# vita-epfl/collaborative-gan-sampling

Hardware: AMD Instinct MI355X
Metric: refined samples/sec @ 20 refinement steps (higher is better)
Workload: dtype f32; 1 GPU; dcgan64 collaborative refinement (propose + K-step refine + render), batch 1024/GPU, K=20, momentum rate 0.1, refine at feature [8, 8, 256], random-init weights, z~U(-1,1) seed 2019+rank; global_batch=1024, refine_steps=20, parallelism=single GPU, hipgraph=True, batches_in_flight=2, fused_per_launch=1, sync_bn=False, contraction=f32

## Files before the change

collaborative-gan-sampling_amd/csrc/api.hip:

```cpp
#include <stdarg.h>
#include <stdio.h>

#include "cgs_internal.h"

static thread_local char g_err[512] = "";
static thread_local const char* g_last_kernel = "";

static thread_local double g_last_flops = 0.0;
static thread_local int g_last_tail[2] = {0, 0};
void cgs_note_tail(int tiles, int split) { g_last_tail[0] = tiles; g_last_tail[1] = split; }
static thread_local int g_contraction = CGS_CONTRACTION_F32;
int cgs_contraction_mode() { return g_contraction; }

void cgs_note_kernel(const char* name) { g_last_kernel = name; }
void cgs_note_flops(double f) { g_last_flops = f; }
void cgs_add_flops(double f) { g_last_flops += f; }

int cgs_set_error(int code, const char* fmt, ...) {
    va_list ap;
    va_start(ap, fmt);
    vsnprintf(g_err, sizeof(g_err), fmt, ap);
    va_end(ap);
    return code;
}

extern "C" {

int cgs_version(void) { return 111; }
const char* cgs_last_error(void) { return g_err; }
const char* cgs_last_kernel(void) { return g_last_kernel; }
double cgs_last_executed_flops(void) { return g_last_flops; }
int cgs_last_tail_tiles(void) { return g_last_tail[0]; }
int cgs_last_tail_split(void) { return g_last_tail[1]; }
int cgs_set_contraction(int mode) {
    if (mode < CGS_CONTRACTION_F32 || mode > CGS_CONTRACTION_BX6_ALL) return cgs_set_error(CGS_EINVAL, "set_contraction: mode %d", mode);
    g_contraction = mode;
    return CGS_OK;
}
int cgs_get_contraction(void) { return g_contraction; }

}

struct ConvCall { CgsLayer L; bool dirT, deconv, bwd; };

static ConvCall conv_call_of(int op, int H, int W, int Cin, int Ho, int Wo, int Cout, int kh, int kw, int sh, int sw) {
    ConvCall c;
    c.deconv = (op == CGS_DECONV_FWD || op == CGS_DECONV_BWD_DATA);
    c.bwd = (op == CGS_CONV_BWD_DATA || op == CGS_DECONV_BWD_DATA);
    c.dirT = (op == CGS_CONV_BWD_DATA || op == CGS_DECONV_FWD);
    CgsLayer& L = c.L;
    L.kh = kh; L.kw = kw; L.sh = sh; L.sw = sw;
    if (!c.deconv) { L.Hb = H; L.Wb = W; L.Cb = Cin; L.Hs = cgs_ceil_div(H, sh > 0 ? sh : 1); L.Ws = cgs_ceil_div(W, sw > 0 ? sw : 1); L.Cs = Cout; }
    else { L.Hs = H; L.Ws = W; L.Cs = Cin; L.Hb = Ho; L.Wb = Wo; L.Cb = Cout; }
    return c;
}

static int check_layer(const CgsLayer& L, const char* who) {
    if (L.kh <= 0 || L.kw <= 0 || L.sh <= 0 || L.sw <= 0 || L.Hb <= 0 || L.Wb <= 0 || L.Cb <= 0 || L.Cs <= 0)
        return cgs_set_error(CGS_EINVAL, "%s: non-positive dimension", who);
    if (L.Hs != cgs_ceil_div(L.Hb, L.sh) || L.Ws != cgs_ceil_div(L.Wb, L.sw))
        return cgs_set_error(CGS_EINVAL, "%s: 'SAME' geometry mismatch: big %dx%d stride %dx%d needs small %dx%d, got %dx%d", who,
                             L.Hb, L.Wb, L.sh, L.sw, cgs_ceil_div(L.Hb, L.sh), cgs_ceil_div(L.Wb, L.sw), L.Hs, L.Ws);
    return CGS_OK;
}

static IgemmParams igemm_geometry(const CgsLayer& L, bool dirT, int B, int epilogue) {
    IgemmParams p{};
    p.B = B; p.epilogue = epilogue;
    if (!dirT) cgs_geom_F(L, p);
    else if (L.sh <= 2 && L.sw <= 2) cgs_geom_T(L, p);
    return p;
}

static size_t in_image_floats(const IgemmParams& p) { return (size_t)p.Hin * p.Win * p.Cred; }
static size_t out_image_floats(const IgemmParams& p) { return (size_t)p.Hout * p.Wout * p.N; }
static size_t images_per_launch(const IgemmParams& p) {
    const size_t in_img = in_image_floats(p) * 4, out_img = out_image_floats(p) * 4;
    return 0x7fffffffUL / (in_img > out_img ? in_img : out_img);
}
static bool whole_batch_in_one_launch(const IgemmParams& p) { return images_per_launch(p) >= (size_t)p.B; }

// ... 429 lines not shown
```

collaborative-gan-sampling_amd/csrc/igemm.hip:

```cpp
#include <stdarg.h>
#include <stdio.h>

#include "cgs_internal.h"
#include "igemm_epilogue.h"

typedef float f32x16 __attribute__((ext_vector_type(16)));

static constexpr int BK = CGS_BK;

void cgs_geom_F(const CgsLayer& L, IgemmParams& p) {
    p.Hin = L.Hb; p.Win = L.Wb; p.Cred = L.Cb;
    p.Hout = L.Hs; p.Wout = L.Ws; p.N = L.Cs; p.Np = cgs_round_up(L.Cs, 64);
    p.S = L.sh; p.So = 1; p.dstep = 1; p.kstep = 1; p.nclasses = 1;
    p.tap_parity = (L.sh == 2 && L.sw == 2 && L.Hs * L.Ws > 64) ? 1 : 0;
    IgemmClass& c = p.cls[0];
    c.R = L.Hs; c.C = L.Ws; c.py = 0; c.px = 0; c.nty = L.kh; c.ntx = L.kw;
    c.dy0 = -cgs_same_pad_before(L.Hb, L.kh, L.sh); c.dx0 = -cgs_same_pad_before(L.Wb, L.kw, L.sw);
    c.ky0 = 0; c.kx0 = 0; c.K = L.kh * L.kw * L.Cb; c.w_off = 0;
    p.vec = (p.Cred % BK) == 0 && c.nty <= 16 && c.ntx <= 16;
}

void cgs_geom_T(const CgsLayer& L, IgemmParams& p) {
    p.Hin = L.Hs; p.Win = L.Ws; p.Cred = L.Cs;
    p.Hout = L.Hb; p.Wout = L.Wb; p.N = L.Cb; p.Np = cgs_round_up(L.Cb, 64);
// ... 22 lines not shown

size_t cgs_packed_floats(const IgemmParams& p) {
    size_t n = 0;
    for (int i = 0; i < p.nclasses; ++i) n += (size_t)cgs_round_up(p.cls[i].K, BK) * p.Np;
    return n;
}

__global__ void pack_weights_kernel(IgemmParams p, const float* __restrict__ w, float* __restrict__ packed,
                                    int kw, int Cb, int Cs, int dirT) {
    const IgemmClass& c = p.cls[blockIdx.y];
    const int Kpad = (c.K + BK - 1) / BK * BK;
    const size_t total = (size_t)Kpad * p.Np;
    for (size_t i = (size_t)blockIdx.x * blockDim.x + threadIdx.x; i < total; i += (size_t)gridDim.x * blockDim.x) {
        const int e = (int)(i & 3);
        const int n = (int)((i >> 2) % p.Np);
        const int k = (int)((i >> 2) / p.Np) * 4 + e;
        float v = 0.f;
        if (k < c.K && n < p.N) {
            int t, ci, ta, tb;
            if (p.vec) {
                const int ntaps = c.nty * c.ntx;
                const int kt = k / BK, chunk = kt / ntaps;
                t = kt - chunk * ntaps; ci = chunk * BK + (k - kt * BK);
                ta = t / c.ntx; tb = t - ta * c.ntx;
                ta = cgs_tap_order(ta, c.nty, p.tap_parity); tb = cgs_tap_order(tb, c.ntx, p.tap_parity);
            } else {
                t = k / p.Cred; ci = k - t * p.Cred;
                ta = t / c.ntx; tb = t - ta * c.ntx;
            }
            const int tap = (c.ky0 + ta * p.kstep) * kw + (c.kx0 + tb * p.kstep);
            const size_t src = dirT ? ((size_t)tap * Cb + n) * Cs + ci
                                    : ((size_t)tap * Cb + ci) * Cs + n;
            v = w[src];
        }
        packed[c.w_off + i] = v;
    }
}

int cgs_pack_weights(const IgemmParams& p, const CgsLayer& L, bool dirT, const float* w, float* packed, hipStream_t s) {
    size_t mx = 0;
    for (int i = 0; i < p.nclasses; ++i) {
        size_t n = (size_t)cgs_round_up(p.cls[i].K, BK) * p.Np;
        if (n > mx) mx = n;
    }
    if (mx == 0) return CGS_OK;
    int blocks = (int)((mx + 255) / 256);
    if (blocks > 4096) blocks = 4096;
    hipLaunchKernelGGL(pack_weights_kernel, dim3(blocks, p.nclasses), dim3(256), 0, s, p, w, packed, L.kw, L.Cb, L.Cs,
                       dirT ? 1 : 0);
    CGS_CHECK_LAUNCH("pack_weights");
    return CGS_OK;
}

template <int BM, int BN, int NW, bool VEC, int TBK, bool PAR, bool NS>
__device__ __forceinline__ void igemm_body(const IgemmParams& p) {
    constexpr int BK = TBK;
    constexpr int LDA = BK + 4;
    constexpr int NT = 64 * NW;
    constexpr int WM = BM / 64;
    constexpr int WN = NW / WM;
    constexpr int TM = BM / (32 * WM), TN = BN / (32 * WN);
    constexpr int QPR = BK / 4;
    constexpr int AI = BM * QPR / NT, BI = BN * QPR / NT;
    constexpr int AR = NT / QPR;
    extern __shared__ __attribute__((aligned(16))) float smem[];
    float* As = smem;
    float* Bs = smem + 2 * BM * LDA;
    constexpr int KLOOP_F = 2 * BM * LDA + 2 * BK * BN;
    constexpr int EH = (VEC && TBK == 16) ? 2 : 1;
    constexpr int STAGE_F = NW * (BM / WM / EH) * (BN / WN + 4);
    int* rowpix = (int*)(smem + (KLOOP_F > STAGE_F ? KLOOP_F : STAGE_F));

    const int nblk_n = p.Np / BN;
    unsigned wi = blockIdx.x;
    int cls_i = blockIdx.y;
    if (p.xcd_map == 2) {
        const unsigned xcd = wi & 7u;
        unsigned q = wi >> 3;
        cls_i = (int)(q % (unsigned)p.nclasses);
        q /= (unsigned)p.nclasses;
        wi = (q << 3) | xcd;
    }
    if (p.cls_flip && (((((unsigned)blockIdx.z * gridDim.y + (unsigned)cls_i) * gridDim.x) >> 8) & 1u)) {
        const int grp = cls_i / p.cls_flip;
        cls_i = grp * p.cls_flip + (p.cls_flip - 1 - (cls_i - grp * p.cls_flip));
    }
    int tsplit = 1, tz = 0, ttile = 0;
    if (p.tail_s > 1 && cls_i == p.nclasses - 1 && wi >= (unsigned)p.tail_from) {
        const unsigned t = wi - (unsigned)p.tail_from;
        ttile = (int)(t / (unsigned)p.tail_s); tz = (int)(t - (unsigned)ttile * (unsigned)p.tail_s); tsplit = p.tail_s;
        if (ttile >= p.tail_n) return;
        wi = (unsigned)p.tail_from + (unsigned)ttile;
    }
    int nb, mb;
    if (p.xcd_map) {
        const unsigned xcd = wi & 7u, q = wi >> 3;
        nb = (int)(q % (unsigned)nblk_n);
        mb = (int)(q / (unsigned)nblk_n) * 8 + (int)xcd;
    } else {
        nb = (int)(wi % (unsigned)nblk_n);
        mb = (int)(wi / (unsigned)nblk_n);
    }
    const IgemmClass& c = p.cls[cls_i];
    const int RC = c.R * c.C;
    const int M = p.B * RC;
    if (mb * BM >= M) return;
    if (p.lpt) {
        const int gpp = p.B / BM;
// ... 77 lines not shown
        return kt < nk ? kt : nk;
    };

    f32x4 ra[AI], rb[BI];
    const __amdgpu_buffer_rsrc_t in_rsrc = __builtin_amdgcn_make_buffer_rsrc(
        (void*)p.in, 0, (int)((unsigned)p.B * (unsigned)p.Hin * (unsigned)p.Win * (unsigned)p.Cred * 4u), 0x00020000);
#define LOAD_TILE(kt_)                                                                                          \
    do {                                                                                                        \
        if constexpr (VEC) {                                                                                    \
            const int kt32_ = TBK == 16 ? (kt_) >> 1 : (kt_);             \
            const int chunk_ = kt32_ / ntaps, t = kt32_ - chunk_ * ntaps;                                       \
            const int ci = chunk_ * 32 + (TBK == 16 ? ((kt_) & 1) * 16 : 0) + aq * 4;                           \
            const int ia_ = t / c.ntx, ib_ = t - ia_ * c.ntx;                                                   \
            const int ta = cgs_tap_order(ia_, c.nty, PAR), tb = cgs_tap_order(ib_, c.ntx, PAR);                 \
            const int dy = ta * p.dstep, dx = tb * p.dstep;                                                     \
            _Pragma("unroll") for (int i = 0; i < AI; ++i) {                                                    \
                const int iy = a_iy[i] + dy, ix = a_ix[i] + dx;                                                 \
                const bool ok = (unsigned)iy < (unsigned)p.Hin && (unsigned)ix < (unsigned)p.Win;               \
                  \
                                              \
                const unsigned off = ok ? (unsigned)((a_base[i] + iy * p.Win + ix) * p.Cred + ci) * 4u : 0xFFFFFFF0u; \
                ra[i] = __builtin_bit_cast(f32x4, __builtin_amdgcn_raw_buffer_load_b128(in_rsrc, off, 0, 0));   \
            }                                                                                                   \
        } else {                                                                                                \
               \
                                    \
            float va[AI][4];                                                                                    \
            _Pragma("unroll") for (int e = 0; e < 4; ++e) {                                                     \
                const int k = (kt_) * BK + aq * 4 + e;                                                          \
                const bool kin = k < c.K;                                                                       \
                const int t = kin ? k / p.Cred : 0, ci = k - t * p.Cred;                                        \
                const int ta = t / c.ntx, tb = t - ta * c.ntx;                                                  \
                const int dy = ta * p.dstep, dx = tb * p.dstep;                                                 \
                _Pragma("unroll") for (int i = 0; i < AI; ++i) {                                                \
                    const int iy = a_iy[i] + dy, ix = a_ix[i] + dx;                                             \
                    const bool ok = kin && (unsigned)iy < (unsigned)p.Hin && (unsigned)ix < (unsigned)p.Win;    \
                    const unsigned off = ok ? (unsigned)((a_base[i] + iy * p.Win + ix) * p.Cred + ci) * 4u : 0xFFFFFFF0u; \
                    va[i][e] = __builtin_bit_cast(float, __builtin_amdgcn_raw_buffer_load_b32(in_rsrc, off, 0, 0)); \
                }                                                                                               \
            }                                                                                                   \
            _Pragma("unroll") for (int i = 0; i < AI; ++i) ra[i] = f32x4{va[i][0], va[i][1], va[i][2], va[i][3]}; \
        }                                                                                                       \
        _Pragma("unroll") for (int i = 0; i < BI; ++i) {                                                        \
            const int idx = tid + NT * i;                                                                       \
            const int kq = idx / BN, n = idx - kq * BN;                                                         \
            rb[i] = *(const f32x4*)(wsrc + ((size_t)((kt_) * (BK / 4) + kq) * p.Np + n0 + n) * 4);            \
        }                                                                                                       \
    } while (0)
#define STORE_TILE(buf_)                                                                                        \
    do {                                                                                                        \
        float* a_ = As + (buf_) * BM * LDA;                                                                     \
        float* b_ = Bs + (buf_) * BK * BN;                                                                      \
        _Pragma("unroll") for (int i = 0; i < AI; ++i) *(f32x4*)(a_ + (ar + AR * i) * LDA + aq * 4) = ra[i];    \
        _Pragma("unroll") for (int i = 0; i < BI; ++i) *(f32x4*)(b_ + (tid + NT * i) * 4) = rb[i];              \
    } while (0)

    f32x16 acc[TM][TN];
#pragma unroll
    for (int tm = 0; tm < TM; ++tm)
#pragma unroll
        for (int tn = 0; tn < TN; ++tn)
#pragma unroll
            for (int r = 0; r < 16; ++r) acc[tm][tn][r] = 0.f;

    struct KIt { int kt, sub, ia, ib, chunk; };
    auto kit_valid = [&](const KIt& s) -> bool {
        if (!skip_ok) return true;
        const int ta = cgs_tap_order(s.ia, c.nty, PAR), tb = cgs_tap_order(s.ib, c.ntx, PAR);
        const int iy = u_iy + ta * p.dstep, ix = u_ix + tb * p.dstep;
        return (unsigned)iy < (unsigned)p.Hin && (unsigned)ix < (unsigned)p.Win;
    };
    auto kit_next_tap = [&](KIt& s) {
        for (;;) {
            if (++s.ib == c.ntx) { s.ib = 0; if (++s.ia == c.nty) { s.ia = 0; ++s.chunk; } }
            if (s.kt >= nk || kit_valid(s)) break;
            s.kt += (TBK == 16 ? 2 : 1);
        }
        if (s.kt > nk) s.kt = nk;
    };
    auto kit_first = [&](int kt0) -> KIt {
        KIt s;
        const int kt32 = (VEC && TBK == 16) ? kt0 >> 1 : kt0;
        s.kt = kt0; s.sub = (VEC && TBK == 16) ? (kt0 & 1) : 0;
        s.chunk = kt32 / ntaps;
        const int t = kt32 - s.chunk * ntaps;
        s.ia = t / c.ntx; s.ib = t - s.ia * c.ntx;
        if (s.kt < nk && !kit_valid(s)) {
            s.kt += (TBK == 16 ? 2 - s.sub : 1); s.sub = 0;
            kit_next_tap(s);
        }
        if (s.kt > nk) s.kt = nk;
        return s;
    };
    auto kit_next = [&](KIt s) -> KIt {
        if (TBK == 16 && s.sub == 0) { s.sub = 1; ++s.kt; if (s.kt > nk) s.kt = nk; return s; }
        s.sub = 0; ++s.kt;
        kit_next_tap(s);
        return s;
    };
    unsigned rowoff[AI], b_voff[BI];
#pragma unroll
    for (int i = 0; i < AI; ++i)
        rowoff[i] = ((unsigned)(a_base[i] + a_iy[i] * p.Win + a_ix[i]) * (unsigned)p.Cred + (unsigned)aq * 4u) * 4u;
#pragma unroll
    for (int i = 0; i < BI; ++i) {
        const int idx = tid + NT * i;
        const int kq = idx / BN, n = idx - kq * BN;
        b_voff[i] = (unsigned)(kq * p.Np + n0 + n) * 16u;
    }
    unsigned tapmask[AI];
    if (one_pix) {
        unsigned mk = 0;
        for (int ia = 0; ia < c.nty; ++ia)
            if ((unsigned)(u_iy + cgs_tap_order(ia, c.nty, PAR) * p.dstep) < (unsigned)p.Hin) mk |= 1u << ia;
        for (int ib = 0; ib < c.ntx; ++ib)
            if ((unsigned)(u_ix + cgs_tap_order(ib, c.ntx, PAR) * p.dstep) < (unsigned)p.Win) mk |= 1u << (16 + ib);
#pragma unroll
        for (int i = 0; i < AI; ++i) tapmask[i] = m0 + ar + AR * i < M ? mk : 0u;
    } else {
#pragma unroll
        for (int i = 0; i < AI; ++i) {
            unsigned mk = 0;
            for (int ia = 0; ia < c.nty; ++ia)
                if ((unsigned)(a_iy[i] + cgs_tap_order(ia, c.nty, PAR) * p.dstep) < (unsigned)p.Hin) mk |= 1u << ia;
            for (int ib = 0; ib < c.ntx; ++ib)
                if ((unsigned)(a_ix[i] + cgs_tap_order(ib, c.ntx, PAR) * p.dstep) < (unsigned)p.Win) mk |= 1u << (16 + ib);
            tapmask[i] = mk;
        }
    }
    const __amdgpu_buffer_rsrc_t w_rsrc = __builtin_amdgcn_make_buffer_rsrc((void*)wsrc, 0, 0x7ffffff0, 0x00020000);
    const int b_tile_bytes = (BK / 4) * p.Np * 16;
    unsigned a_off[AI];
#define ADDR_TILE_V(s_)                                                                                         \
    do {                                                                                                        \
        const int ta_ = cgs_tap_order((s_).ia, c.nty, PAR), tb_ = cgs_tap_order((s_).ib, c.ntx, PAR);           \
        const int dy_ = ta_ * p.dstep, dx_ = tb_ * p.dstep;                                                     \
        const unsigned soff_ = (unsigned)(((dy_ * p.Win + dx_) * p.Cred + (s_).chunk * 32 + (TBK == 16 ? (s_).sub * 16 : 0)) * 4); \
        const unsigned need_ = (1u << (s_).ia) | (1u << (16 + (s_).ib));                                        \
        _Pragma("unroll") for (int i = 0; i < AI; ++i)                                                          \
            a_off[i] = (tapmask[i] & need_) == need_ ? rowoff[i] + soff_ : 0xFFFFFFF0u;                         \
    } while (0)
#define ISSUE_TILE_V(s_)                                                                                        \
    do {                                                                                                        \
        _Pragma("unroll") for (int i = 0; i < AI; ++i)                                                          \
            ra[i] = __builtin_bit_cast(f32x4, __builtin_amdgcn_raw_buffer_load_b128(in_rsrc, a_off[i], 0, 0));  \
        const int b_soff_ = (s_).kt * b_tile_bytes;                                                             \
        _Pragma("unroll") for (int i = 0; i < BI; ++i)                                                          \
            rb[i] = __builtin_bit_cast(f32x4, __builtin_amdgcn_raw_buffer_load_b128(w_rsrc, b_voff[i], b_soff_, 0)); \
    } while (0)

    const bool uni = VEC && p.uni && skip_ok && m0 + BM <= M;
    unsigned rowoff_u[AI];
#pragma unroll
    for (int i = 0; i < AI; ++i) rowoff_u[i] = ((unsigned)a_base[i] * (unsigned)p.Cred + (unsigned)aq * 4u) * 4u;
    unsigned a_soff = 0;
#define ADDR_TILE_U(s_)                                                                                         \
    do {                                                                                                        \
        const int ta_ = cgs_tap_order((s_).ia, c.nty, PAR), tb_ = cgs_tap_order((s_).ib, c.ntx, PAR);           \
        const int iy_ = u_iy + ta_ * p.dstep, ix_ = u_ix + tb_ * p.dstep;                                       \
        a_soff = (unsigned)(((iy_ * p.Win + ix_) * p.Cred + (s_).chunk * 32 + (TBK == 16 ? (s_).sub * 16 : 0)) * 4); \
    } while (0)
#define ISSUE_TILE_U(s_)                                                                                        \
    do {                                                                                                        \
        _Pragma("unroll") for (int i = 0; i < AI; ++i)                                                          \
            ra[i] = __builtin_bit_cast(f32x4, __builtin_amdgcn_raw_buffer_load_b128(in_rsrc, rowoff_u[i], a_soff, 0)); \
        const int b_soff_ = (s_).kt * b_tile_bytes;                                                             \
        _Pragma("unroll") for (int i = 0; i < BI; ++i)                                                          \
            rb[i] = __builtin_bit_cast(f32x4, __builtin_amdgcn_raw_buffer_load_b128(w_rsrc, b_voff[i], b_soff_, 0)); \
    } while (0)

    KIt cur;
    int kt;
    if constexpr (VEC) {
        cur = kit_first(kbeg);
        kt = cur.kt;
        if (cur.kt < nk) {
            ADDR_TILE_V(cur);
            ISSUE_TILE_V(cur);
            STORE_TILE(0);
        }
    } else {
        kt = next_chunk(kbeg);
        cur.kt = kt;
        if (kt < nk) {
            LOAD_TILE(kt);
            STORE_TILE(0);
        }
    }
    __syncthreads();

#define MFMA_GROUP(jj_)                                                                                         \
    do {                                                                                                        \
        const int kq = 2 * (jj_) + h;                                                                           \
        f32x4 fa[TM], fb[TN];                                                                                   \
        _Pragma("unroll") for (int tm = 0; tm < TM; ++tm) fa[tm] = *(const f32x4*)(a + tm * 32 * LDA + kq * 4); \
        _Pragma("unroll") for (int tn = 0; tn < TN; ++tn) fb[tn] = *(const f32x4*)(b + (kq * BN + tn * 32) * 4); \
        _Pragma("unroll") for (int tm = 0; tm < TM; ++tm)                                                       \
            _Pragma("unroll") for (int tn = 0; tn < TN; ++tn) {                                                 \
                acc[tm][tn] = __builtin_amdgcn_mfma_f32_32x32x2f32(fa[tm].x, fb[tn].x, acc[tm][tn], 0, 0, 0);   \
                acc[tm][tn] = __builtin_amdgcn_mfma_f32_32x32x2f32(fa[tm].y, fb[tn].y, acc[tm][tn], 0, 0, 0);   \
                acc[tm][tn] = __builtin_amdgcn_mfma_f32_32x32x2f32(fa[tm].z, fb[tn].z, acc[tm][tn], 0, 0, 0);   \
                acc[tm][tn] = __builtin_amdgcn_mfma_f32_32x32x2f32(fa[tm].w, fb[tn].w, acc[tm][tn], 0, 0, 0);   \
            }                                                                                                   \
    } while (0)
    constexpr int NG = BK / 8;
    int pt1 = 1 << 30, pt2 = 1 << 30;
    if (p.prio_t[0] > 0) {
        const int span = nk - kbeg;
        pt1 = kbeg + ((span * p.prio_t[0]) >> 8); pt2 = kbeg + ((span * p.prio_t[1]) >> 8);
        __builtin_amdgcn_s_setprio(2);
    } else {
        __builtin_amdgcn_s_setprio(0);
    }
#define PRIO_STEP(kt_)                                                                                          \
    if ((kt_) >= pt1) {                       \
        if ((kt_) >= pt2) { __builtin_amdgcn_s_setprio(0); pt1 = 1 << 30; }                                     \
        else { __builtin_amdgcn_s_setprio(1); pt1 = pt2; }                                                      \
    }

#define FRAG_READ(buf_, jj_, fa_, fb_)                                                                          \
    do {                                                                                                        \
        const float* a_ = As + (buf_) * BM * LDA + (wm * (BM / WM) + j) * LDA;                                   \
        const float* b_ = Bs + (buf_) * BK * BN + (wn * (BN / WN) + j) * 4;                                     \
        const int kq = 2 * (jj_) + h;                                                                           \
        _Pragma("unroll") for (int tm = 0; tm < TM; ++tm) fa_[tm] = *(const f32x4*)(a_ + tm * 32 * LDA + kq * 4); \
        _Pragma("unroll") for (int tn = 0; tn < TN; ++tn) fb_[tn] = *(const f32x4*)(b_ + (kq * BN + tn * 32) * 4); \
    } while (0)
#define MFMA_EXEC(fa_, fb_)                                                                                     \
    do {                                                                                                        \
        _Pragma("unroll") for (int tm = 0; tm < TM; ++tm)                                                       \
            _Pragma("unroll") for (int tn = 0; tn < TN; ++tn) {                                                 \
                acc[tm][tn] = __builtin_amdgcn_mfma_f32_32x32x2f32(fa_[tm].x, fb_[tn].x, acc[tm][tn], 0, 0, 0); \
                acc[tm][tn] = __builtin_amdgcn_mfma_f32_32x32x2f32(fa_[tm].y, fb_[tn].y, acc[tm][tn], 0, 0, 0); \
                acc[tm][tn] = __builtin_amdgcn_mfma_f32_32x32x2f32(fa_[tm].z, fb_[tn].z, acc[tm][tn], 0, 0, 0); \
                acc[tm][tn] = __builtin_amdgcn_mfma_f32_32x32x2f32(fa_[tm].w, fb_[tn].w, acc[tm][tn], 0, 0, 0); \
            }                                                                                                   \
    } while (0)
    if constexpr (VEC && TBK == 32) {
        f32x4 fa0[TM], fb0[TN], fa1[TM], fb1[TN];
#define KIT_SEL(d_, c_, a_, b_)                                                                                 \
    do {                                                                                                        \
        const bool c__ = (c_);                                                                                  \
        d_.kt = c__ ? a_.kt : b_.kt; d_.sub = c__ ? a_.sub : b_.sub; d_.ia = c__ ? a_.ia : b_.ia;               \
        d_.ib = c__ ? a_.ib : b_.ib; d_.chunk = c__ ? a_.chunk : b_.chunk;                                      \
    } while (0)
#define K_LOOP32(ADDR_, ISSUE_)                                                                                 \
    {                                                                                                           \
        KIt nxt = cur, ld = cur;                                                                                \
        if (cur.kt < nk) nxt = kit_next(cur);                                                                   \
        KIT_SEL(ld, nxt.kt < nk, nxt, cur);           \
        if (cur.kt < nk) {                                                                                      \
            FRAG_READ(0, 0, fa0, fb0);                                                                          \
            ADDR_(ld);                                                                                          \
        }                                                                                                       \
        for (int buf = 0; cur.kt < nk; buf ^= 1) {                                                              \
            ISSUE_(ld);                                                                                         \
            _Pragma("unroll") for (int jj = 0; jj + 1 < NG; jj += 2) {      \
                FRAG_READ(buf, jj + 1, fa1, fb1);                                                               \
                __builtin_amdgcn_sched_barrier(0);                                                              \
                MFMA_EXEC(fa0, fb0);                                                                            \
                __builtin_amdgcn_sched_barrier(0);                                                              \
                if (jj + 2 < NG) {                                                                              \
                    FRAG_READ(buf, jj + 2, fa0, fb0);                                                           \
                    __builtin_amdgcn_sched_barrier(0);                                                          \
                    MFMA_EXEC(fa1, fb1);                                                                        \
                    __builtin_amdgcn_sched_barrier(0);                                                          \
                }                                                                                               \
            }                                                                                                   \
            STORE_TILE(buf ^ 1);                                                                                \
            __syncthreads();                                                                                    \
            FRAG_READ(buf ^ 1, 0, fa0, fb0);          \
            __builtin_amdgcn_sched_barrier(0);                                                                  \
                              \
            cur = nxt;                                                                                          \
            if (cur.kt < nk) {                                                                                  \
                nxt = kit_next(cur);                                                                            \
                KIT_SEL(ld, nxt.kt < nk, nxt, cur);                                                             \
            }                                                                                                   \
            ADDR_(ld);                                                                                          \
            MFMA_EXEC(fa1, fb1);                                                                                \
            __builtin_amdgcn_sched_barrier(0);                                                                  \
        }                                                                                                       \
    }
        if (uni) K_LOOP32(ADDR_TILE_U, ISSUE_TILE_U)
        else K_LOOP32(ADDR_TILE_V, ISSUE_TILE_V)
#undef K_LOOP32
    } else if constexpr (VEC) {
#define TILE_BODY(BUF_, NXT_, ADDR_, ISSUE_)                                                                   \
    {                                                                                                           \
        PRIO_STEP(cur.kt);                                                                                      \
        KIt ld = NXT_;                                   \
        if ((NXT_).kt >= nk) ld = cur;                                                                          \
        const float* a = As + (BUF_) * BM * LDA + (wm * (BM / WM) + j) * LDA;                                    \
        const float* b = Bs + (BUF_) * BK * BN + (wn * (BN / WN) + j) * 4;                                      \
        MFMA_GROUP(0);                                                                                          \
        ADDR_(ld);                                                                                              \
        ISSUE_(ld);                                                                                             \
        _Pragma("unroll") for (int jj = 1; jj < NG - 1; ++jj) MFMA_GROUP(jj);                                   \
        STORE_TILE((BUF_) ^ 1);                                                                                 \
        if (NG > 1) MFMA_GROUP(NG - 1);                                                                         \
        __syncthreads();                                                                                        \
        cur = NXT_;                                                                                             \
    }
#define K_LOOP16(ADDR_, ISSUE_)                                                                                 \
    {                                                                                                           \
        KIt n1 = cur;                                                                                           \
        if (cur.kt < nk) n1 = kit_next(cur);                                                                    \
        while (n1.kt < nk) {                              \
            const KIt n2 = kit_next(n1);                                                                        \
            KIt n3 = n2;                                                                                        \
            if (n2.kt < nk) n3 = kit_next(n2);                                                                  \
            TILE_BODY(0, n1, ADDR_, ISSUE_);                                                                    \
            TILE_BODY(1, n2, ADDR_, ISSUE_);                                                                    \
            n1 = n3;                                                                                            \
        }                                                                                                       \
        if (cur.kt < nk) {                                                                \
            TILE_BODY(0, n1, ADDR_, ISSUE_);                                                                    \
        }                                                                                                       \
    }
        if (uni) K_LOOP16(ADDR_TILE_U, ISSUE_TILE_U)
        else K_LOOP16(ADDR_TILE_V, ISSUE_TILE_V)
#undef K_LOOP16
#undef TILE_BODY
    } else {
        for (int buf = 0; kt < nk; buf ^= 1) {
            const int kn = next_chunk(kt + 1);
            const int kl = kn < nk ? kn : kt;
            const float* a = As + buf * BM * LDA + (wm * (BM / WM) + j) * LDA;
            const float* b = Bs + buf * BK * BN + (wn * (BN / WN) + j) * 4;
            MFMA_GROUP(0);
            LOAD_TILE(kl);
#pragma unroll
            for (int jj = 1; jj < NG - 1; ++jj) MFMA_GROUP(jj);
            STORE_TILE(buf ^ 1);
            if (NG > 1) MFMA_GROUP(NG - 1);
            __syncthreads();
            kt = kn;
        }
    }
#undef KIT_SEL
#undef FRAG_READ
#undef MFMA_EXEC
#undef ADDR_TILE_V
#undef ISSUE_TILE_V
#undef ADDR_TILE_U
#undef ISSUE_TILE_U
#undef PRIO_STEP
#undef MFMA_GROUP

#undef LOAD_TILE
#undef STORE_TILE
#undef DECODE_ROW
    __builtin_amdgcn_s_setprio(3);
    if (tsplit > 1) {
        float* slab = p.slab + ((size_t)ttile * tsplit + tz) * (BM * BN);
#pragma unroll
        for (int tn = 0; tn < TN; ++tn) {
            const int nl = wn * (BN / WN) + tn * 32 + j;
#pragma unroll
            for (int tm = 0; tm < TM; ++tm)
#pragma unroll
                for (int r = 0; r < 16; ++r) {
                    const int ml = wm * (BM / WM) + tm * 32 + (r & 3) + 8 * (r >> 2) + 4 * h;
                    slab[ml * BN + nl] = acc[tm][tn][r];
                }
        }
        return;
    }
    if (p.splitk > 1) {
        float* slab = p.slab + c.slab_off + (size_t)blockIdx.z * M * p.Np;
#pragma unroll
        for (int tn = 0; tn < TN; ++tn) {
            const int n = n0 + wn * (BN / WN) + tn * 32 + j;
#pragma unroll
            for (int tm = 0; tm < TM; ++tm)
#pragma unroll
                for (int r = 0; r < 16; ++r) {
                    const int m = m0 + wm * (BM / WM) + tm * 32 + (r & 3) + 8 * (r >> 2) + 4 * h;
                    if (m < M) slab[(size_t)m * p.Np + n] = acc[tm][tn][r];
                }
        }
        return;
    }
    constexpr int WTN = BN / WN;
    if ((p.N & 3) == 0) {
        constexpr int LDE = WTN + 4;
        constexpr int ER = BM / WM / EH;
        float* E = smem + wave * ER * LDE;
        constexpr int LPR = WTN / 4;
        constexpr int RPP = 64 / LPR;
        const int c4 = (lane % LPR) * 4, rsub = lane / LPR;
        const int n = n0 + wn * WTN + c4;
        f32x4 bias = {0.f, 0.f, 0.f, 0.f}, ea = {1.f, 1.f, 1.f, 1.f}, eb = {0.f, 0.f, 0.f, 0.f};
        if (n < p.N) {
            if (p.bias) bias = *(const f32x4*)(p.bias + n);
            if (p.epilogue == CGS_EPI_AFFINE_RELU) { ea = *(const f32x4*)(p.ep_a + n); eb = *(const f32x4*)(p.ep_b + n); }
            if (p.epilogue == CGS_EPI_RELU_BWD_AFFINE) ea = *(const f32x4*)(p.ep_a + n);
        }
        f32x4 st_a = {0.f, 0.f, 0.f, 0.f}, st_b = {0.f, 0.f, 0.f, 0.f};
// ... 25 lines not shown
                switch (p.epilogue) {
                    case CGS_EPI_NONE: epilogue_rows<CGS_EPI_NONE, ER, RPP, LDE>(p, E, rp, rsub, c4, n, bias, ea, eb); break;
                    case CGS_EPI_LRELU: epilogue_rows<CGS_EPI_LRELU, ER, RPP, LDE>(p, E, rp, rsub, c4, n, bias, ea, eb); break;
                    case CGS_EPI_AFFINE_RELU: epilogue_rows<CGS_EPI_AFFINE_RELU, ER, RPP, LDE>(p, E, rp, rsub, c4, n, bias, ea, eb); break;
                    case CGS_EPI_TANH: epilogue_rows<CGS_EPI_TANH, ER, RPP, LDE>(p, E, rp, rsub, c4, n, bias, ea, eb); break;
                    case CGS_EPI_RELU_BWD_AFFINE: epilogue_rows<CGS_EPI_RELU_BWD_AFFINE, ER, RPP, LDE>(p, E, rp, rsub, c4, n, bias, ea, eb); break;
                    case CGS_EPI_LRELU_BWD: epilogue_rows<CGS_EPI_LRELU_BWD, ER, RPP, LDE>(p, E, rp, rsub, c4, n, bias, ea, eb); break;
                    default: epilogue_rows<CGS_EPI_TANH_BWD, ER, RPP, LDE>(p, E, rp, rsub, c4, n, bias, ea, eb); break;
                }
            }
            if (ph + 1 < EH) {
                __builtin_amdgcn_fence(__ATOMIC_RELEASE, "wavefront");
                __builtin_amdgcn_wave_barrier();
                __builtin_amdgcn_fence(__ATOMIC_ACQUIRE, "wavefront");
            }
        }
        if (p.stat_part) {
#pragma unroll
            for (int off = LPR; off < 64; off <<= 1)
#pragma unroll
                for (int e = 0; e < 4; ++e) { st_a[e] += __shfl_xor(st_a[e], off); st_b[e] += __shfl_xor(st_b[e], off); }
            if (rsub == 0 && n < p.N) {
                float* dst = p.stat_part + ((size_t)(cls_i * p.stat_cls_rows + m0 / 64 + wm) * 2) * p.N + n;
                *(f32x4*)dst = st_a;
                *(f32x4*)(dst + p.N) = st_b;
            }
        }
        return;
    }
#pragma unroll
    for (int tn = 0; tn < TN; ++tn) {
        const int n = n0 + wn * WTN + tn * 32 + j;
        if (n >= p.N) continue;
        const float bias = p.bias ? p.bias[n] : 0.f;
        float ea = 1.f, eb = 0.f;
        if (p.epilogue == CGS_EPI_AFFINE_RELU) { ea = p.ep_a[n]; eb = p.ep_b[n]; }
        if (p.epilogue == CGS_EPI_RELU_BWD_AFFINE) ea = p.ep_a[n];
        const bool use_aux = p.epilogue >= CGS_EPI_RELU_BWD_AFFINE;
#pragma unroll
        for (int tm = 0; tm < TM; ++tm)
#pragma unroll
            for (int r = 0; r < 16; ++r) {
                const int row = wm * (BM / WM) + tm * 32 + (r & 3) + 8 * (r >> 2) + 4 * h;
                const int pix = rowpix[row];
                if (pix >= 0) {
                    const size_t o = (size_t)pix * p.N + n;
                    const float aux = use_aux ? p.ep_aux[o] : 0.f;
                    p.out[o] = epilogue_apply(acc[tm][tn][r] + bias, p.epilogue, ea, eb, aux);
                }
            }
    }
}

template <int BM, int BN, int NW, bool VEC, int TBK, bool PAR>
__global__ __launch_bounds__(64 * NW, 2) void igemm_kernel(IgemmParams p) { igemm_body<BM, BN, NW, VEC, TBK, PAR, false>(p); }
template <int BM, int BN, int NW, bool VEC, int TBK, bool PAR>
__global__ __launch_bounds__(64 * NW, 2) void igemm_ns_kernel(IgemmParams p) { igemm_body<BM, BN, NW, VEC, TBK, PAR, true>(p); }

__global__ __launch_bounds__(256) void splitk_reduce_kernel(IgemmParams p) {
    const IgemmClass& c = p.cls[blockIdx.y];
    const int RC = c.R * c.C;
    const int M = p.B * RC;
    const int nq = p.Np / 4;
    const long total = (long)M * nq;
    const float* slab = p.slab + c.slab_off;
    const int g = threadIdx.x & 3;
    const long stride = (long)gridDim.x * (blockDim.x >> 2);
    const long total_pad = (total + stride - 1) / stride * stride;
    for (long i = (long)blockIdx.x * (blockDim.x >> 2) + (threadIdx.x >> 2); i < total_pad; i += stride) {
        const bool live = i < total;
        const int m = live ? (int)(i / nq) : 0, n = live ? (int)(i - (long)m * nq) * 4 : 0;
        f32x4 a = {0.f, 0.f, 0.f, 0.f};
        if (live)
            for (int sidx = g; sidx < p.splitk; sidx += 4) a += *(const f32x4*)(slab + ((size_t)sidx * M + m) * p.Np + n);
#pragma unroll
        for (int e = 0; e < 4; ++e) {
            a[e] += __shfl_xor(a[e], 1);
            a[e] += __shfl_xor(a[e], 2);
        }
        if (!live || g != 0) continue;
        int b, r, cc, rem;
        if (p.pix_major) { rem = m / p.B; b = m - rem * p.B; } else { b = m / RC; rem = m - b * RC; }
        r = rem / c.C; cc = rem - r * c.C;
        const size_t o = (size_t)((b * p.Hout + r * p.So + c.py) * p.Wout + cc * p.So + c.px) * p.N;
#pragma unroll
        for (int e = 0; e < 4; ++e) {
            if (n + e >= p.N) break;
            const float bias = p.bias ? p.bias[n + e] : 0.f;
            float ea = 1.f, eb = 0.f;
            if (p.epilogue == CGS_EPI_AFFINE_RELU) { ea = p.ep_a[n + e]; eb = p.ep_b[n + e]; }
            if (p.epilogue == CGS_EPI_RELU_BWD_AFFINE) ea = p.ep_a[n + e];
            const float aux = p.epilogue >= CGS_EPI_RELU_BWD_AFFINE ? p.ep_aux[o + n + e] : 0.f;
            p.out[o + n + e] = epilogue_apply(a[e] + bias, p.epilogue, ea, eb, aux);
        }
    }
}

__global__ __launch_bounds__(256) void splitk_reduce_stats_kernel(IgemmParams p) {
    const int cls_i = blockIdx.z;
    const IgemmClass& c = p.cls[cls_i];
    const int RC = c.R * c.C;
    const int M = p.B * RC;
    const float* slab = p.slab + c.slab_off;
    const int cq = threadIdx.x & 7, rl = threadIdx.x >> 3;
    const int n = blockIdx.y * 32 + cq * 4;
    __shared__ f32x4 red[2][32][8];
    f32x4 sa = {0.f, 0.f, 0.f, 0.f}, sb = {0.f, 0.f, 0.f, 0.f};
    if (n < p.N) {
        f32x4 bias = {0.f, 0.f, 0.f, 0.f};
        if (p.bias) bias = *(const f32x4*)(p.bias + n);
// ... 86 lines not shown
        for (int e = 0; e < 4; ++e) y[e] = epilogue_apply(a[e] + bias[e], p.epilogue, ea[e], eb[e], aux[e]);
        *(f32x4*)(p.out + o) = y;
    }
}

static long igemm_blocks(const IgemmParams& p, int BN, int BM = 128) {
    long blocks = 0;
    for (int i = 0; i < p.nclasses; ++i) blocks += (((long)p.B * p.cls[i].R * p.cls[i].C + BM - 1) / BM) * (p.Np / BN);
    return blocks;
}

static int choose_splitk(const IgemmParams& p) {
    const int BN = (p.Np % 128) == 0 ? 128 : 64;
    const long blocks = igemm_blocks(p, BN);
    int nk_min = 1 << 30;
    for (int i = 0; i < p.nclasses; ++i) {
        const int nk = cgs_ceil_div(p.cls[i].K, BK);
        if (p.cls[i].R * p.cls[i].C > 0 && nk < nk_min) nk_min = nk;
    }
    if (blocks == 0 || blocks >= 256 || nk_min < 8) return 1;
    long cap = nk_min / 4;
    if (cap > 64) cap = 64;
    if (cap < 2) return 1;
    int nk_max = 0;
    double slice_mb = 0.0;
    long maxM = 0;
    for (int i = 0; i < p.nclasses; ++i) {
        const long m = (long)p.B * p.cls[i].R * p.cls[i].C;
        if (m <= 0) continue;
        const int nk = cgs_ceil_div(p.cls[i].K, BK);
        if (nk > nk_max) nk_max = nk;
        if (m > maxM) maxM = m;
        slice_mb += (double)m * p.Np * 4e-6;
    }
    const double tile = (BN == 128 ? 1.0 : 0.5) * (maxM <= 64 ? 0.5 : 1.0);
    int best = 1;
    double best_cost = 1e30;
    for (long s = 2; s <= cap; ++s) {
        const long cps = (nk_max + s - 1) / s;
        if ((nk_max + cps - 1) / cps != s) continue;
        const long load = (blocks * s + 255) / 256;
        const double cost = (load == 1 ? 1.41 : (double)load) * (double)cps * tile + 0.3 * slice_mb * (double)s;
        if (cost < best_cost) { best_cost = cost; best = (int)s; }
    }
    return best;
}

struct IgemmTiles { bool wide, mid, deep, tall, wide_for_tail; };
struct IgemmTail { int from, n, s; };
static IgemmTail igemm_choose_tail(const IgemmParams& p, const IgemmTiles& t);

#define IGEMM_CUS 256
static bool igemm_round_rules_apply() {
    static int cus = -1;
    if (cus < 0) {
        int dev = 0, n = 0;
        if (hipGetDevice(&dev) != hipSuccess || hipDeviceGetAttribute(&n, hipDeviceAttributeMultiprocessorCount, dev) != hipSuccess) n = 0;
        cus = n;
    }
    return cus == IGEMM_CUS || cus == 0;
}

static IgemmTiles igemm_choose_tiles(const IgemmParams& p, bool tail_wide = true) {
    const bool vec = p.vec != 0;
    int maxRC = 0;
    for (int i = 0; i < p.nclasses; ++i) maxRC = p.cls[i].R * p.cls[i].C > maxRC ? p.cls[i].R * p.cls[i].C : maxRC;
    bool wide = (p.Np % 128) == 0, wide_for_tail = false;
    if (wide && p.lpt && maxRC <= 64) {
        long blocks = 0;
        for (int i = 0; i < p.nclasses; ++i) blocks += ((long)p.B * p.cls[i].R * p.cls[i].C / 128) * (p.Np / 128);
        if (blocks < 1024) wide = false;
        if (!wide && tail_wide && vec && p.splitk == 1 && !p.stat_part && !p.sign_out && (p.N & 3) == 0 && p.nclasses == 1 && blocks >= 512 && blocks <= 1024 &&
            (blocks % 256) != 0 && (blocks % 256) <= 176 && igemm_choose_tail(p, IgemmTiles{true, false, false, false, true}).s > 1) {
            wide = true;
            wide_for_tail = true;
        }
    }
    bool mid = false;
    if (wide && vec && p.splitk == 1) {
        const long wb = igemm_blocks(p, 128);
        if (wb >= 256 && wb < 512) { wide = false; mid = true; }
        else if (wb < 256 && (p.stat_part || p.sign_out)) { wide = false; mid = true; }
    }
    bool deep = true;
    if (vec && p.splitk == 1 && !mid) {
        long min_blocks = 1L << 40, tot_blocks = 0;
        for (int i = 0; i < p.nclasses; ++i) {
            const long m = (long)p.B * p.cls[i].R * p.cls[i].C;
            if (m > 0) { const long bl = (m + 127) / 128 * (p.Np / (wide ? 128 : 64)); if (bl < min_blocks) min_blocks = bl; tot_blocks += bl; }
        }
        deep = min_blocks < 512;
        if (deep && !p.pix_major && p.nclasses > 1 && tot_blocks >= 1024) deep = false;
    }
    bool tall = false;
    {
        int kmax = 0;
        for (int i = 0; i < p.nclasses; ++i) kmax = p.cls[i].K > kmax ? p.cls[i].K : kmax;
        tall = vec && !wide && !mid && !deep && p.splitk == 1 && p.Np == 64 && p.pix_major && (p.B % 256) == 0 && kmax <= 512 &&
               igemm_blocks(p, 64, 256) >= 1536;
    }
    return IgemmTiles{wide, mid, deep, tall, wide_for_tail && wide};
}

static int igemm_blocks_per_cu(bool wide, bool deep) { return deep ? (wide ? 2 : 3) : (wide ? 4 : 5); }

static IgemmTail igemm_choose_tail(const IgemmParams& p, const IgemmTiles& t) {
    IgemmTail none{0, 0, 0};
    if (!igemm_round_rules_apply()) return none;
    if (!p.vec || p.splitk > 1 || p.stat_part || p.sign_out || (p.N & 3) || t.tall) return none;
    const int bn = t.wide ? 128 : 64, tbk = t.deep ? 32 : 16;
    const IgemmClass& cl = p.cls[p.nclasses - 1];
    const long Ml = (long)p.B * cl.R * cl.C;
    if (Ml <= 0) return none;
    const long mtl = (Ml + 127) / 128, Tl = mtl * (p.Np / bn);
    const long T = igemm_blocks(p, bn);
    const long L = 256L * igemm_blocks_per_cu(t.wide, t.deep);
    const int nk = cgs_ceil_div(cl.K, tbk);
    if (T < 256) return none;
    if (T > L) return none;
    long r = T % 256;
    if (r == 0 || r > 176) return none;
    int S = (int)((256 + r / 2) / r);
    if (S > 16) S = 16;
    if (S > nk / 4) S = nk / 4;
    if (S < 2) return none;
    if (r > Tl) r = Tl;
    for (int i = 0; i < p.nclasses; ++i)
        if ((long)p.B * p.cls[i].R * p.cls[i].C != Ml) return none;
    const bool xcd_map = (mtl % 8 == 0 || mtl >= 64);
    const long ids = (xcd_map ? (mtl + 7) / 8 * 8 : mtl) * (p.Np / bn);
    if (xcd_map && (mtl % 8) != 0) return none;
    return IgemmTail{(int)(ids - r), (int)r, S};
}

static size_t igemm_tail_bytes(const IgemmTail& tl, bool wide) { return (size_t)tl.n * tl.s * 128 * (wide ? 128 : 64) * sizeof(float); }

size_t cgs_igemm_slab_bytes(const IgemmParams& p_in) {
    const size_t sk = cgs_igemm_splitk_bytes(p_in);
    if (sk) return sk;
    IgemmParams p = p_in;
    p.splitk = 1; p.stat_part = nullptr; p.sign_out = nullptr;
    cgs_igemm_row_policy(p, 128);
    const IgemmTiles t = igemm_choose_tiles(p);
    const IgemmTail tl = igemm_choose_tail(p, t);
    return tl.s > 1 ? igemm_tail_bytes(tl, t.wide) : 0;
}

int cgs_igemm_signs_ok(const IgemmParams& p) {
    return (p.N % 32) == 0 && (p.epilogue == CGS_EPI_AFFINE_RELU || p.epilogue == CGS_EPI_LRELU) && choose_splitk(p) <= 1;
}

size_t cgs_igemm_splitk_bytes(const IgemmParams& p) {
    const int s = choose_splitk(p);
    if (s <= 1) return 0;
    size_t n = 0;
    for (int i = 0; i < p.nclasses; ++i) n += (size_t)s * p.B * p.cls[i].R * p.cls[i].C * p.Np;
    return n * sizeof(float);
}

template <int BM, int BN, int NW, bool VEC, int TBK, bool PAR, bool NS>
static int launch_cfg(const IgemmParams& p, hipStream_t s) {
    void (*const kern)(IgemmParams) = NS ? igemm_ns_kernel<BM, BN, NW, VEC, TBK, PAR> : igemm_kernel<BM, BN, NW, VEC, TBK, PAR>;
    constexpr int EH = (VEC && TBK == 16) ? 2 : 1;
    constexpr int WM = BM / 64;
    constexpr size_t kloop_f = (size_t)2 * BM * (TBK + 4) + 2 * TBK * BN, stage_f = (size_t)NW * (BM / WM / EH) * (BN / (NW / WM) + 4);
    constexpr size_t smem = (kloop_f > stage_f ? kloop_f : stage_f) * sizeof(float) + BM * sizeof(int);
    static bool attr_done[64] = {};
    int dev_ = 0;
    (void)hipGetDevice(&dev_);
    dev_ &= 63;
    if (!attr_done[dev_]) {
        hipError_t e = hipFuncSetAttribute((const void*)kern, hipFuncAttributeMaxDynamicSharedMemorySize, (int)smem);
        if (e != hipSuccess) return cgs_set_error(CGS_ELAUNCH, "igemm smem attr: %s", hipGetErrorString(e));
        attr_done[dev_] = true;
    }
    long maxM = 0;
    for (int i = 0; i < p.nclasses; ++i) {
        long m = (long)p.B * p.cls[i].R * p.cls[i].C;
        if (m > maxM) maxM = m;
    }
    if (maxM == 0) return CGS_OK;
    const long mtiles = (maxM + BM - 1) / BM;
    IgemmParams q = p;
    q.xcd_map = (mtiles % 8 == 0 || mtiles >= 64) ? 1 : 0;
    long gx = (q.xcd_map ? (mtiles + 7) / 8 * 8 : mtiles) * (p.Np / BN);
    if (p.tail_s > 1) {
        if ((long)p.tail_from + p.tail_n != gx) return cgs_set_error(CGS_EINVAL, "igemm: tail split planned for another grid (%d + %d != %ld)", p.tail_from, p.tail_n, gx);
        gx = (long)p.tail_from + (long)p.tail_n * p.tail_s;
    }
    unsigned gy = (unsigned)p.nclasses;
    {
        const long total = gx * (long)p.nclasses * (p.splitk > 1 ? p.splitk : 1);
        q.cls_flip = 0;
        if (igemm_round_rules_apply() && p.nclasses > 1 && !p.pix_major && total > 256 && total <= 512 && gx > 0 && (256 % gx) == 0 && p.tail_s <= 1) {
            const long per_round = 256 / gx;
            if (p.splitk > 1 && (per_round % p.nclasses) == 0) q.cls_flip = p.nclasses;
            else if (p.splitk == 1 && per_round < p.nclasses && (p.nclasses % per_round) == 0) q.cls_flip = (int)per_round;
        }
    }
    if (gx > 0x7fffffffL) return cgs_set_error(CGS_EINVAL, "igemm: grid too large");
    hipLaunchKernelGGL(kern, dim3((unsigned)gx, gy, p.splitk > 1 ? p.splitk : 1), dim3(64 * NW), smem, s, q);
    CGS_CHECK_LAUNCH("igemm");
    if (p.tail_s > 1) {
        hipLaunchKernelGGL(tail_reduce_kernel, dim3((unsigned)p.tail_n, TAIL_RSPLIT), dim3(256), 0, s, q, BM, BN);
        CGS_CHECK_LAUNCH("tail_reduce");
    }
    if (p.splitk > 1) {
        long tot = 0;
        for (int i = 0; i < p.nclasses; ++i) { long t = (long)p.B * p.cls[i].R * p.cls[i].C * (p.Np / 4); if (t > tot) tot = t; }
        unsigned rb = (unsigned)((tot + 63) / 64 > 4096 ? 4096 : (tot + 63) / 64);
        if (p.stat_part) hipLaunchKernelGGL(splitk_reduce_stats_kernel, dim3((unsigned)p.stat_cls_rows, (unsigned)((p.N + 31) / 32), p.nclasses), dim3(256), 0, s, p);
        else hipLaunchKernelGGL(splitk_reduce_kernel, dim3(rb, p.nclasses), dim3(256), 0, s, p);
        CGS_CHECK_LAUNCH("splitk_reduce");
    }
    static char name[64];
// ... 96 lines not shown
    }
    const bool vec = p.vec != 0;
    IgemmTiles tiles = igemm_choose_tiles(p);
    IgemmTail tl = igemm_choose_tail(p, tiles);
    bool tail_fits = tl.s > 1 && slab && slab_bytes >= igemm_tail_bytes(tl, tiles.wide);
    if (tiles.wide_for_tail && !tail_fits) {
        tiles = igemm_choose_tiles(p, false);
        tl = igemm_choose_tail(p, tiles);
        tail_fits = tl.s > 1 && slab && slab_bytes >= igemm_tail_bytes(tl, tiles.wide);
    }
    bool wide = tiles.wide, deep = tiles.deep;
    const bool tall = tiles.tall;
    if (tall) cgs_igemm_row_policy(p, 256);
    cgs_igemm_count_flops(p, tall ? 256 : 128);
    if (tail_fits) {
        p.tail_from = tl.from; p.tail_n = tl.n; p.tail_s = tl.s; p.slab = (float*)slab;
        cgs_note_tail(tl.n, tl.s);
    }
    {
        const int bn_sel = wide ? 128 : 64, per_cu = vec ? igemm_blocks_per_cu(wide, deep) : 2;
        const long total_blocks = igemm_blocks(p, bn_sel);
        const bool one_round = igemm_round_rules_apply() && vec && p.splitk == 1 && !tall && total_blocks <= (long)IGEMM_CUS * per_cu && total_blocks >= IGEMM_CUS;
        if (vec && !deep && p.splitk == 1 && p.pix_major && total_blocks >= 256) { p.prio_t[0] = 85; p.prio_t[1] = 170; p.prio_t[2] = 0; }
        const int nblk_n = p.Np / bn_sel;
        if (one_round && p.lpt && p.nclasses == 1 && p.B / 128 == 8 && (32 % nblk_n) == 0) {
            const IgemmClass& c = p.cls[0];
            const int RC = c.R * c.C, nbins = 32 / nblk_n, cap = (RC + nbins - 1) / nbins;
            int cnt[256], load[32] = {}, used[32] = {};
            unsigned char bin_items[32][256];
            for (int pix = 0; pix < RC; ++pix) {
                const int r = pix / c.C, cc = pix - r * c.C;
                int ny = 0, nx = 0;
                for (int ta = 0; ta < c.nty; ++ta) { const int iy = r * p.S + c.dy0 + ta * p.dstep; ny += (iy >= 0 && iy < p.Hin); }
                for (int tb = 0; tb < c.ntx; ++tb) { const int ix = cc * p.S + c.dx0 + tb * p.dstep; nx += (ix >= 0 && ix < p.Win); }
                cnt[pix] = ny * nx;
            }
            for (int i = 0; i < RC; ++i) {
                const int pix = p.perm[0][i];
                int best = -1;
                for (int b = 0; b < nbins; ++b) {
                    const int slots = (RC - b + nbins - 1) / nbins;
                    if (used[b] < slots && used[b] < cap && (best < 0 || load[b] < load[best])) best = b;
                }
                bin_items[best][used[best]++] = (unsigned char)pix;
                load[best] += cnt[pix];
            }
            for (int b = 0; b < nbins; ++b)
                for (int k = 0; k < used[b]; ++k) p.perm[0][b + k * nbins] = bin_items[b][k];
        }
    }
    p.uni = !(p.nclasses > 1 && wide && maxRC <= 64);
    bool half = vec && wide && deep && p.splitk > 1 && !p.tap_parity && (long)p.B * maxRC <= 64;
    const bool ns = p.stat_part && p.ns_mean;
#define LC(...) (ns ? launch_cfg<__VA_ARGS__, true>(p, s) : launch_cfg<__VA_ARGS__, false>(p, s))
    if (half) return LC(64, 128, 4, true, 32, false);
    if (tall) return p.tap_parity ? LC(256, 64, 4, true, 16, true) : LC(256, 64, 4, true, 16, false);
    if (vec && !deep && !p.tap_parity) return wide ? LC(128, 128, 4, true, 16, false) : LC(128, 64, 4, true, 16, false);
    if (vec && !deep && p.tap_parity) return wide ? LC(128, 128, 4, true, 16, true) : LC(128, 64, 4, true, 16, true);
    if (vec && p.tap_parity) return wide ? LC(128, 128, 4, true, 32, true) : LC(128, 64, 4, true, 32, true);
    if (vec) return wide ? LC(128, 128, 4, true, 32, false) : LC(128, 64, 4, true, 32, false);
    return wide ? LC(128, 128, 4, false, 16, false) : LC(128, 64, 4, false, 16, false);
#undef LC
}
```

Measured before the change: 6745 samples/s.

## Load igemm weight tiles directly into LDS via buffer_load_lds for selected configs

```diff
diff --git a/collaborative-gan-sampling_amd/csrc/api.hip b/collaborative-gan-sampling_amd/csrc/api.hip
--- a/collaborative-gan-sampling_amd/csrc/api.hip
+++ b/collaborative-gan-sampling_amd/csrc/api.hip
@@ -26,7 +26,7 @@
 
 extern "C" {
 
-int cgs_version(void) { return 111; }
+int cgs_version(void) { return 112; }
 const char* cgs_last_error(void) { return g_err; }
 const char* cgs_last_kernel(void) { return g_last_kernel; }
 double cgs_last_executed_flops(void) { return g_last_flops; }
diff --git a/collaborative-gan-sampling_amd/csrc/igemm.hip b/collaborative-gan-sampling_amd/csrc/igemm.hip
--- a/collaborative-gan-sampling_amd/csrc/igemm.hip
+++ b/collaborative-gan-sampling_amd/csrc/igemm.hip
@@ -98,8 +98,9 @@
     return CGS_OK;
 }
 
-template <int BM, int BN, int NW, bool VEC, int TBK, bool PAR, bool NS>
+template <int BM, int BN, int NW, bool VEC, int TBK, bool PAR, bool NS, bool BDMA>
 __device__ __forceinline__ void igemm_body(const IgemmParams& p) {
+    static_assert(!BDMA || VEC, "the direct weight load serves the VEC kernels only");
     constexpr int BK = TBK;
     constexpr int LDA = BK + 4;
     constexpr int NT = 64 * NW;
@@ -283,7 +284,9 @@
         float* a_ = As + (buf_) * BM * LDA;                                                                     \
         float* b_ = Bs + (buf_) * BK * BN;                                                                      \
         _Pragma("unroll") for (int i = 0; i < AI; ++i) *(f32x4*)(a_ + (ar + AR * i) * LDA + aq * 4) = ra[i];    \
-        _Pragma("unroll") for (int i = 0; i < BI; ++i) *(f32x4*)(b_ + (tid + NT * i) * 4) = rb[i];              \
+        if constexpr (!BDMA) {                        \
+            _Pragma("unroll") for (int i = 0; i < BI; ++i) *(f32x4*)(b_ + (tid + NT * i) * 4) = rb[i];          \
+        }                                                                                                       \
     } while (0)
 
     f32x16 acc[TM][TN];
@@ -361,6 +364,8 @@
     }
     const __amdgpu_buffer_rsrc_t w_rsrc = __builtin_amdgcn_make_buffer_rsrc((void*)wsrc, 0, 0x7ffffff0, 0x00020000);
     const int b_tile_bytes = (BK / 4) * p.Np * 16;
+    typedef __attribute__((address_space(3))) void* lds_ptr_t;
+    float* const b_lds = Bs + __builtin_amdgcn_readfirstlane(wave) * 64 * 4;
     unsigned a_off[AI];
 #define ADDR_TILE_V(s_)                                                                                         \
     do {                                                                                                        \
@@ -371,13 +376,22 @@
         _Pragma("unroll") for (int i = 0; i < AI; ++i)                                                          \
             a_off[i] = (tapmask[i] & need_) == need_ ? rowoff[i] + soff_ : 0xFFFFFFF0u;                         \
     } while (0)
-#define ISSUE_TILE_V(s_)                                                                                        \
+#define ISSUE_B(s_, dst_)                                                                                       \
     do {                                                                                                        \
+        const int b_soff_ = (s_).kt * b_tile_bytes;                                                             \
+        if constexpr (BDMA) {                                                                                   \
+            _Pragma("unroll") for (int i = 0; i < BI; ++i)                                                      \
+                __builtin_amdgcn_raw_ptr_buffer_load_lds(w_rsrc, (lds_ptr_t)(b_lds + (dst_) * BK * BN + NT * i * 4), 16, b_voff[i], b_soff_, 0, 0); \
+        } else {                                                                                                \
+            _Pragma("unroll") for (int i = 0; i < BI; ++i)                                                      \
+                rb[i] = __builtin_bit_cast(f32x4, __builtin_amdgcn_raw_buffer_load_b128(w_rsrc, b_voff[i], b_soff_, 0)); \
+        }                                                                                                       \
+    } while (0)
+#define ISSUE_TILE_V(s_, dst_)                                                                                  \
+    do {                                                                                                        \
+        ISSUE_B(s_, dst_);                                                                                      \
         _Pragma("unroll") for (int i = 0; i < AI; ++i)                                                          \
             ra[i] = __builtin_bit_cast(f32x4, __builtin_amdgcn_raw_buffer_load_b128(in_rsrc, a_off[i], 0, 0));  \
-        const int b_soff_ = (s_).kt * b_tile_bytes;                                                             \
-        _Pragma("unroll") for (int i = 0; i < BI; ++i)                                                          \
-            rb[i] = __builtin_bit_cast(f32x4, __builtin_amdgcn_raw_buffer_load_b128(w_rsrc, b_voff[i], b_soff_, 0)); \
     } while (0)
 
     const bool uni = VEC && p.uni && skip_ok && m0 + BM <= M;
@@ -391,13 +405,16 @@
         const int iy_ = u_iy + ta_ * p.dstep, ix_ = u_ix + tb_ * p.dstep;                                       \
         a_soff = (unsigned)(((iy_ * p.Win + ix_) * p.Cred + (s_).chunk * 32 + (TBK == 16 ? (s_).sub * 16 : 0)) * 4); \
     } while (0)
-#define ISSUE_TILE_U(s_)                                                                                        \
+#define ISSUE_TILE_U(s_, dst_)                                                                                  \
     do {                                                                                                        \
+        ISSUE_B(s_, dst_);                                                                                      \
         _Pragma("unroll") for (int i = 0; i < AI; ++i)                                                          \
             ra[i] = __builtin_bit_cast(f32x4, __builtin_amdgcn_raw_buffer_load_b128(in_rsrc, rowoff_u[i], a_soff, 0)); \
-        const int b_soff_ = (s_).kt * b_tile_bytes;                                                             \
-        _Pragma("unroll") for (int i = 0; i < BI; ++i)                                                          \
-            rb[i] = __builtin_bit_cast(f32x4, __builtin_amdgcn_raw_buffer_load_b128(w_rsrc, b_voff[i], b_soff_, 0)); \
+    } while (0)
+
+#define DMA_WAIT()                                                                                              \
+    do {                                                                                                        \
+        if constexpr (BDMA) asm volatile("s_waitcnt vmcnt(0) lgkmcnt(0)" ::: "memory");                         \
     } while (0)
 
     KIt cur;
@@ -407,7 +424,7 @@
         kt = cur.kt;
         if (cur.kt < nk) {
             ADDR_TILE_V(cur);
-            ISSUE_TILE_V(cur);
+            ISSUE_TILE_V(cur, 0);
             STORE_TILE(0);
         }
     } else {
@@ -418,6 +435,7 @@
             STORE_TILE(0);
         }
     }
+    DMA_WAIT();
     __syncthreads();
 
 #define MFMA_GROUP(jj_)                                                                                         \
@@ -485,7 +503,7 @@
             ADDR_(ld);                                                                                          \
         }                                                                                                       \
         for (int buf = 0; cur.kt < nk; buf ^= 1) {                                                              \
-            ISSUE_(ld);                                                                                         \
+            ISSUE_(ld, buf ^ 1);                                                                                \
             _Pragma("unroll") for (int jj = 0; jj + 1 < NG; jj += 2) {      \
                 FRAG_READ(buf, jj + 1, fa1, fb1);                                                               \
                 __builtin_amdgcn_sched_barrier(0);                                                              \
@@ -499,6 +517,7 @@
                 }                                                                                               \
             }                                                                                                   \
             STORE_TILE(buf ^ 1);                                                                                \
+            DMA_WAIT();                                                                                         \
             __syncthreads();                                                                                    \
             FRAG_READ(buf ^ 1, 0, fa0, fb0);          \
             __builtin_amdgcn_sched_barrier(0);                                                                  \
@@ -526,10 +545,11 @@
         const float* b = Bs + (BUF_) * BK * BN + (wn * (BN / WN) + j) * 4;                                      \
         MFMA_GROUP(0);                                                                                          \
         ADDR_(ld);                                                                                              \
-        ISSUE_(ld);                                                                                             \
+        ISSUE_(ld, (BUF_) ^ 1);                                                                                 \
         _Pragma("unroll") for (int jj = 1; jj < NG - 1; ++jj) MFMA_GROUP(jj);                                   \
         STORE_TILE((BUF_) ^ 1);                                                                                 \
         if (NG > 1) MFMA_GROUP(NG - 1);                                                                         \
+        DMA_WAIT();                                                                                             \
         __syncthreads();                                                                                        \
         cur = NXT_;                                                                                             \
     }
@@ -576,6 +596,8 @@
 #undef ISSUE_TILE_V
 #undef ADDR_TILE_U
 #undef ISSUE_TILE_U
+#undef ISSUE_B
+#undef DMA_WAIT
 #undef PRIO_STEP
 #undef MFMA_GROUP
 
@@ -707,10 +729,10 @@
     }
 }
 
-template <int BM, int BN, int NW, bool VEC, int TBK, bool PAR>
-__global__ __launch_bounds__(64 * NW, 2) void igemm_kernel(IgemmParams p) { igemm_body<BM, BN, NW, VEC, TBK, PAR, false>(p); }
-template <int BM, int BN, int NW, bool VEC, int TBK, bool PAR>
-__global__ __launch_bounds__(64 * NW, 2) void igemm_ns_kernel(IgemmParams p) { igemm_body<BM, BN, NW, VEC, TBK, PAR, true>(p); }
+template <int BM, int BN, int NW, bool VEC, int TBK, bool PAR, bool BDMA>
+__global__ __launch_bounds__(64 * NW, 2) void igemm_kernel(IgemmParams p) { igemm_body<BM, BN, NW, VEC, TBK, PAR, false, BDMA>(p); }
+template <int BM, int BN, int NW, bool VEC, int TBK, bool PAR, bool BDMA>
+__global__ __launch_bounds__(64 * NW, 2) void igemm_ns_kernel(IgemmParams p) { igemm_body<BM, BN, NW, VEC, TBK, PAR, true, BDMA>(p); }
 
 __global__ __launch_bounds__(256) void splitk_reduce_kernel(IgemmParams p) {
     const IgemmClass& c = p.cls[blockIdx.y];
@@ -903,12 +925,16 @@
 
 #define IGEMM_CUS 256
 static bool igemm_round_rules_apply() {
-    static int cus = -1;
-    if (cus < 0) {
-        int dev = 0, n = 0;
-        if (hipGetDevice(&dev) != hipSuccess || hipDeviceGetAttribute(&n, hipDeviceAttributeMultiprocessorCount, dev) != hipSuccess) n = 0;
-        cus = n;
-    }
+    static int cus_of[64];
+    int dev = 0;
+    if (hipGetDevice(&dev) != hipSuccess) return true;
+    dev &= 63;
+    if (cus_of[dev] == 0) {
+        int n = 0;
+        if (hipDeviceGetAttribute(&n, hipDeviceAttributeMultiprocessorCount, dev) != hipSuccess || n < 0) n = 0;
+        cus_of[dev] = n + 1;
+    }
+    const int cus = cus_of[dev] - 1;
     return cus == IGEMM_CUS || cus == 0;
 }
 
@@ -1009,9 +1035,13 @@
     return n * sizeof(float);
 }
 
-template <int BM, int BN, int NW, bool VEC, int TBK, bool PAR, bool NS>
+static constexpr bool igemm_b_direct(int BM, int BN, bool VEC, int TBK, bool PAR) {
+    return VEC && BM == 128 && ((TBK == 16 && !PAR) || (TBK == 32 && BN == 64));
+}
+
+template <int BM, int BN, int NW, bool VEC, int TBK, bool PAR, bool NS, bool BDMA>
 static int launch_cfg(const IgemmParams& p, hipStream_t s) {
-    void (*const kern)(IgemmParams) = NS ? igemm_ns_kernel<BM, BN, NW, VEC, TBK, PAR> : igemm_kernel<BM, BN, NW, VEC, TBK, PAR>;
+    void (*const kern)(IgemmParams) = NS ? igemm_ns_kernel<BM, BN, NW, VEC, TBK, PAR, BDMA> : igemm_kernel<BM, BN, NW, VEC, TBK, PAR, BDMA>;
     constexpr int EH = (VEC && TBK == 16) ? 2 : 1;
     constexpr int WM = BM / 64;
     constexpr size_t kloop_f = (size_t)2 * BM * (TBK + 4) + 2 * TBK * BN, stage_f = (size_t)NW * (BM / WM / EH) * (BN / (NW / WM) + 4);
@@ -1214,7 +1244,10 @@
     p.uni = !(p.nclasses > 1 && wide && maxRC <= 64);
     bool half = vec && wide && deep && p.splitk > 1 && !p.tap_parity && (long)p.B * maxRC <= 64;
     const bool ns = p.stat_part && p.ns_mean;
-#define LC(...) (ns ? launch_cfg<__VA_ARGS__, true>(p, s) : launch_cfg<__VA_ARGS__, false>(p, s))
+#define LC_(BM_, BN_, NW_, VEC_, TBK_, PAR_) \
+    (ns ? launch_cfg<BM_, BN_, NW_, VEC_, TBK_, PAR_, true, igemm_b_direct(BM_, BN_, VEC_, TBK_, PAR_)>(p, s) \
+        : launch_cfg<BM_, BN_, NW_, VEC_, TBK_, PAR_, false, igemm_b_direct(BM_, BN_, VEC_, TBK_, PAR_)>(p, s))
+#define LC(...) LC_(__VA_ARGS__)
     if (half) return LC(64, 128, 4, true, 32, false);
     if (tall) return p.tap_parity ? LC(256, 64, 4, true, 16, true) : LC(256, 64, 4, true, 16, false);
     if (vec && !deep && !p.tap_parity) return wide ? LC(128, 128, 4, true, 16, false) : LC(128, 64, 4, true, 16, false);
@@ -1223,4 +1256,5 @@
     if (vec) return wide ? LC(128, 128, 4, true, 32, false) : LC(128, 64, 4, true, 32, false);
     return wide ? LC(128, 128, 4, false, 16, false) : LC(128, 64, 4, false, 16, false);
 #undef LC
-}
+#undef LC_
+}
```

Result: no change. 6740 samples/s (-0.1%).
